# Chatit-cloud/BEE2BEE

Measured on NVIDIA H100. Metric: decode_tokens_per_sec, higher is better.
Workload: dtype bf16

## Files before the change

csrc/attention_tc.cu:

```cuda
#include "kernels.h"

#include <cuda.h>
#include <cuda_fp8.h>

#include <cstdlib>
#include <type_traits>

#include "common.cuh"
#include "launch.cuh"
#include "wgmma.cuh"

namespace b2b {

int make_tmap_shared(CUtensorMap* m, const void* ptr, uint64_t rows, uint64_t cols, uint64_t ld, uint32_t box_rows,
                     int elt_bytes);

namespace {

constexpr int APAGE = 64;
constexpr int ATC_CONSUMERS = 256;
constexpr int ATC_THREADS = ATC_CONSUMERS + 32;
constexpr float LOG2E = 1.4426950408889634f;

struct AttnTcParams {
  __nv_bfloat16* out;
  const int* block_table;
  const int* q_start;
  const int* q_len;
  const int* kv_len;
  int max_pages, n_q, n_kv, window;
  float softcap;
  int splits, ws_rows;
  float* ws;
  uint8_t* q_out8;
  uint8_t* q_sf;
  int q_bn;
};

template <int D>
struct AtcCfg {
  static constexpr int BKV = 64;
  static constexpr int kQBytes = 128 * D * 2;
  static constexpr int kKVBytes = BKV * D * 2;
  static constexpr int kSmemBytes = kQBytes + 4 * kKVBytes + 256;
};

template <int D, bool SOFTCAP>
__global__ void __launch_bounds__(ATC_THREADS, 1)
attn_prefill_tc_kernel(const __grid_constant__ CUtensorMap tm_q, const __grid_constant__ CUtensorMap tm_k,
                       const __grid_constant__ CUtensorMap tm_v, const AttnTcParams p, const int G, const int QB) {
  using Cfg = AtcCfg<D>;
  constexpr int BKV = Cfg::BKV;
  constexpr int DB = D / 64;

  extern __shared__ __align__(1024) uint8_t smem[];
  if ((smem_u32(smem) & 1023u) != 0u) __trap();
  uint8_t* q_s = smem;
  uint8_t* k_s = q_s + Cfg::kQBytes;
  uint8_t* v_s = k_s + 2 * Cfg::kKVBytes;
  uint64_t* bars = reinterpret_cast<uint64_t*>(v_s + 2 * Cfg::kKVBytes);
  uint64_t* q_full = bars + 0;
  uint64_t* k_full = bars + 1;
  uint64_t* v_full = bars + 3;
  uint64_t* k_empty = bars + 5;
  uint64_t* v_empty = bars + 7;

  const int warp = threadIdx.x >> 5, lane = threadIdx.x & 31;
  if (threadIdx.x == ATC_CONSUMERS) {
    mbar_init(q_full, 1);
    for (int i = 0; i < 2; ++i) {
      mbar_init(&k_full[i], 1); mbar_init(&v_full[i], 1);
      mbar_init(&k_empty[i], ATC_CONSUMERS / 32); mbar_init(&v_empty[i], ATC_CONSUMERS / 32);
    }
    fence_barrier_init();
    tma_prefetch_desc(&tm_q); tma_prefetch_desc(&tm_k); tma_prefetch_desc(&tm_v);
  }
  __syncthreads();

  pdl_launch_dependents();
  pdl_wait();
  const int seq = blockIdx.z, kvh = blockIdx.y;
  const bool split_mode = p.splits > 1;
  const int qblk = split_mode ? 0 : gridDim.x - 1 - blockIdx.x;
  const int qlen = p.q_len[seq], kvlen = p.kv_len[seq];
  const int q0 = qblk * QB;
  bool active = q0 < qlen;
  const int nq_here = min(QB, qlen - q0);
  const int qtok0 = p.q_start[seq] + q0;
  const int pos0 = kvlen - qlen + q0;
  const int kv_hi = min(kvlen, pos0 + nq_here);
  const int kv_lo = p.window > 0 ? max(0, pos0 - p.window + 1) : 0;
  int t_lo = kv_lo / BKV, t_hi = (kv_hi + BKV - 1) / BKV;
  if (active && split_mode) {
    const int per = (t_hi - t_lo + p.splits - 1) / p.splits;
    t_lo = min(t_hi, t_lo + static_cast<int>(blockIdx.x) * per);
    t_hi = min(t_hi, t_lo + per);
    if (t_hi <= t_lo) {
      if (threadIdx.x < G) {
        float* w = p.ws + (((static_cast<size_t>(seq) * p.n_kv + kvh) * p.splits + blockIdx.x) * p.ws_rows + threadIdx.x) * (D + 2);
        for (int c = 0; c < D; ++c) w[c] = 0.f;
        w[D] = -INFINITY;
        w[D + 1] = 0.f;
      }
      active = false;
    }
  }
  const int nt = t_hi - t_lo;
  if (!active) return;

  if (warp == ATC_CONSUMERS / 32) {
    if (lane == 0) {
      mbar_arrive_expect_tx(q_full, Cfg::kQBytes);
      for (int g = 0; g < G; ++g)
        for (int c = 0; c < DB; ++c)
          tma_load_2d(q_s + c * (128 * 128) + g * QB * 128, &tm_q, q_full, (kvh * G + g) * D + c * 64, qtok0);
      const int* bt = p.block_table + static_cast<size_t>(seq) * p.max_pages;
      for (int n = 0; n < nt; ++n) {
        const int s = n & 1;
        const uint32_t ph = static_cast<uint32_t>((n >> 1) & 1);
        const int page = bt[t_lo + n];
        mbar_wait(&k_empty[s], ph ^ 1u);
        mbar_arrive_expect_tx(&k_full[s], Cfg::kKVBytes);
#pragma unroll
        for (int c = 0; c < DB; ++c)
          tma_load_2d(k_s + s * Cfg::kKVBytes + c * (BKV * 128), &tm_k, &k_full[s], kvh * D + c * 64, page * APAGE);
        mbar_wait(&v_empty[s], ph ^ 1u);
        mbar_arrive_expect_tx(&v_full[s], Cfg::kKVBytes);
#pragma unroll
        for (int c = 0; c < DB; ++c)
          tma_load_2d(v_s + s * Cfg::kKVBytes + c * (BKV * 128), &tm_v, &v_full[s], kvh * D + c * 64, page * APAGE);
      }
    }
    return;
  }

  const int wg = warp >> 2;
  const int ra = wg * 64 + (warp & 3) * 16 + (lane >> 2);
  int gq[2], iq[2], qpos[2];
  bool valid[2];
#pragma unroll
  for (int h = 0; h < 2; ++h) {
    const int row = ra + 8 * h;
    gq[h] = row / QB;
    iq[h] = row % QB;
    valid[h] = (gq[h] < G) && (iq[h] < nq_here);
    qpos[h] = pos0 + iq[h];
  }
  const float cap = p.softcap;
  const float inv_cap = SOFTCAP ? 1.f / cap : 0.f;
  float m_ref[2] = {-INFINITY, -INFINITY}, l[2] = {0.f, 0.f};
  float o[D / 2];
#pragma unroll
  for (int e = 0; e < D / 2; ++e) o[e] = 0.f;
  auto release = [&](uint64_t* bar) {
    __syncwarp();
    if (lane == 0) mbar_arrive(bar);
  };

  mbar_wait(q_full, 0);
  auto tile = [&](int n, auto masked) {
    const int t = t_lo + n, s = n & 1;
    const uint32_t ph = static_cast<uint32_t>((n >> 1) & 1);
    float sc[BKV / 2];
#pragma unroll
    for (int e = 0; e < BKV / 2; ++e) sc[e] = 0.f;
    mbar_wait(&k_full[s], ph);
    wgmma_fence();
#pragma unroll
    for (int kk = 0; kk < D / 16; ++kk) {
      const uint64_t a = make_sw128_kmajor_desc(smem_u32(q_s + (kk / 4) * (128 * 128) + wg * 64 * 128)) +
                         static_cast<uint64_t>((kk % 4) * 2);
      const uint64_t b = make_sw128_kmajor_desc(smem_u32(k_s + s * Cfg::kKVBytes + (kk / 4) * (BKV * 128))) +
                         static_cast<uint64_t>((kk % 4) * 2);
      Wgmma<BKV>::bf16_ss(sc, a, b, kk > 0 ? 1u : 0u);
    }
    wgmma_commit();
    wgmma_wait<0>();
    wgmma_fence_regs(sc);
    release(&k_empty[s]);

    float mrow[2] = {-INFINITY, -INFINITY};
#pragma unroll
    for (int e = 0; e < BKV / 2; ++e) {
      const int h = (e >> 1) & 1;
      float v = sc[e];
      if constexpr (SOFTCAP) v = cap * tanhf(v * inv_cap);
      v *= LOG2E;
      if constexpr (decltype(masked)::value) {
        const int kvpos = t * BKV + (e >> 2) * 8 + 2 * (lane & 3) + (e & 1);
        const bool ok = valid[h] && kvpos <= qpos[h] && kvpos < kvlen && (p.window <= 0 || kvpos > qpos[h] - p.window);
        v = ok ? v : -INFINITY;
      }
      sc[e] = v;
      mrow[h] = fmaxf(mrow[h], v);
    }
    float alpha[2], mr[2];
#pragma unroll
    for (int h = 0; h < 2; ++h) {
      mrow[h] = fmaxf(mrow[h], __shfl_xor_sync(0xffffffffu, mrow[h], 1));
      mrow[h] = fmaxf(mrow[h], __shfl_xor_sync(0xffffffffu, mrow[h], 2));
      alpha[h] = 1.f;
      if (mrow[h] > m_ref[h] + 8.f || (m_ref[h] == -INFINITY && mrow[h] > -INFINITY)) {
        alpha[h] = (m_ref[h] == -INFINITY) ? 0.f : exp2f(m_ref[h] - mrow[h]);
        m_ref[h] = mrow[h];
      }
      mr[h] = (m_ref[h] == -INFINITY) ? 0.f : m_ref[h];
    }
#pragma unroll
    for (int e = 0; e < D / 2; ++e) o[e] *= alpha[(e >> 1) & 1];
    uint32_t pa[BKV / 16][4];
    float lsum[2] = {0.f, 0.f};
#pragma unroll
    for (int e = 0; e < BKV / 2; e += 2) {
      const int h = (e >> 1) & 1;
      const float p0 = exp2f(sc[e] - mr[h]), p1 = exp2f(sc[e + 1] - mr[h]);
      lsum[h] += p0 + p1;
      const __nv_bfloat162 hv = __floats2bfloat162_rn(p0, p1);
      pa[e / 8][(e % 8) / 2] = *reinterpret_cast<const uint32_t*>(&hv);
    }
    l[0] = l[0] * alpha[0] + lsum[0];
    l[1] = l[1] * alpha[1] + lsum[1];
    mbar_wait(&v_full[s], ph);
    wgmma_fence_regs(o);
    wgmma_fence();
#pragma unroll
    for (int kk = 0; kk < BKV / 16; ++kk) {
      const uint64_t b = make_sw128_mnmajor_desc(smem_u32(v_s + s * Cfg::kKVBytes + kk * (16 * 128)), BKV * 128);
      Wgmma<D>::bf16_rs_tb(o, pa[kk], b, 1u);
    }
    wgmma_commit();
    wgmma_wait<0>();
    wgmma_fence_regs(o);
    release(&v_empty[s]);
  };

  for (int n = 0; n < nt; ++n) {
    const int t = t_lo + n;
    const bool full = nq_here == QB && (t + 1) * BKV - 1 <= pos0 && (t + 1) * BKV <= kvlen &&
                      (p.window <= 0 || t * BKV > pos0 + nq_here - 1 - p.window);
    if (full) tile(n, std::false_type{}); else tile(n, std::true_type{});
  }

#pragma unroll
  for (int h = 0; h < 2; ++h) {
    l[h] += __shfl_xor_sync(0xffffffffu, l[h], 1);
    l[h] += __shfl_xor_sync(0xffffffffu, l[h], 2);
  }
  const int c2 = 2 * (lane & 3);
#pragma unroll
  for (int h = 0; h < 2; ++h) {
    const float inv = l[h] > 0.f ? 1.f / l[h] : 0.f;
    const int tok = qtok0 + iq[h], head = kvh * G + gq[h];
    if (split_mode) {
      if (valid[h]) {
        float* wsrow = p.ws + (((static_cast<size_t>(seq) * p.n_kv + kvh) * p.splits + blockIdx.x) * p.ws_rows + gq[h]) * (D + 2);
        if ((lane & 3) == 0) {
          wsrow[D] = (m_ref[h] == -INFINITY) ? -INFINITY : m_ref[h] * 0.6931471805599453f;
          wsrow[D + 1] = l[h];
        }
#pragma unroll
        for (int j = 0; j < D / 8; ++j)
          *reinterpret_cast<float2*>(wsrow + 8 * j + c2) = make_float2(o[4 * j + 2 * h], o[4 * j + 2 * h + 1]);
      }
    } else if (p.q_out8 != nullptr) {
      const int ldq = p.n_q * D;
#pragma unroll
      for (int b = 0; b < D / 32; ++b) {
        float v[8];
        float amax = 0.f;
#pragma unroll
        for (int jj = 0; jj < 4; ++jj) {
          v[2 * jj] = bf16_round(o[4 * (4 * b + jj) + 2 * h] * inv);
          v[2 * jj + 1] = bf16_round(o[4 * (4 * b + jj) + 2 * h + 1] * inv);
          amax = fmaxf(amax, fmaxf(fabsf(v[2 * jj]), fabsf(v[2 * jj + 1])));
        }
        amax = fmaxf(amax, __shfl_xor_sync(0xffffffffu, amax, 1));
        amax = fmaxf(amax, __shfl_xor_sync(0xffffffffu, amax, 2));
        const uint32_t u = __float_as_uint(amax * (1.f / 448.f));
        int ex = static_cast<int>(u >> 23) - 127 + ((u & 0x7FFFFFu) ? 1 : 0);
        ex = max(-126, min(127, ex));
        const float scl = __uint_as_float(static_cast<uint32_t>(127 - ex) << 23);
        if (valid[h]) {
          const int feat = head * D + 32 * b;
          uint8_t* q8 = p.q_out8 + static_cast<size_t>(tok) * ldq + feat;
#pragma unroll
          for (int jj = 0; jj < 4; ++jj) {
            const uint16_t lo = __nv_cvt_float_to_fp8(v[2 * jj] * scl, __NV_SATFINITE, __NV_E4M3);
            const uint16_t hi = __nv_cvt_float_to_fp8(v[2 * jj + 1] * scl, __NV_SATFINITE, __NV_E4M3);
            *reinterpret_cast<uint16_t*>(q8 + 8 * jj + c2) = static_cast<uint16_t>(lo | (hi << 8));
          }
          if ((lane & 3) == 0) {
            const int tile_i = tok / p.q_bn, n = tok - tile_i * p.q_bn, rr = n & 127;
            p.q_sf[(static_cast<size_t>(tile_i) * (ldq >> 7) + (feat >> 7)) * (p.q_bn > 128 ? 1024 : 512) + (n >> 7) * 512 +
                   (rr & 31) * 16 + (rr >> 5) * 4 + ((feat >> 5) & 3)] = static_cast<uint8_t>(ex + 127);
          }
        }
      }
    } else if (valid[h]) {
      __nv_bfloat16* dst = p.out + (static_cast<size_t>(tok) * p.n_q + head) * D;
#pragma unroll
      for (int j = 0; j < D / 8; ++j)
        *reinterpret_cast<__nv_bfloat162*>(dst + 8 * j + c2) =
            __floats2bfloat162_rn(o[4 * j + 2 * h] * inv, o[4 * j + 2 * h + 1] * inv);
    }
  }
}

template <int D, bool SOFTCAP>
int launch_tc_cap(const CUtensorMap& tq, const CUtensorMap& tk, const CUtensorMap& tv, const AttnTcParams& p, int G, int QB,
                  int seqs, int qblocks, cudaStream_t s) {
  using Cfg = AtcCfg<D>;
  static bool set[64] = {};
  int dev = 0;
  cudaGetDevice(&dev);
  if (dev < 64 && !set[dev]) {
    cudaError_t e = cudaFuncSetAttribute(attn_prefill_tc_kernel<D, SOFTCAP>, cudaFuncAttributeMaxDynamicSharedMemorySize,
                                         Cfg::kSmemBytes);
    if (e != cudaSuccess) return static_cast<int>(e);
    set[dev] = true;
  }
  return static_cast<int>(launch_kernel(attn_prefill_tc_kernel<D, SOFTCAP>,
                                        dim3(p.splits > 1 ? p.splits : qblocks, p.n_kv, seqs), dim3(ATC_THREADS),
                                        Cfg::kSmemBytes, s, 1, tq, tk, tv, p, G, QB));
}

template <int D>
int launch_tc(const CUtensorMap& tq, const CUtensorMap& tk, const CUtensorMap& tv, const AttnTcParams& p, int G, int QB,
              int seqs, int qblocks, cudaStream_t s) {
  return p.softcap > 0.f ? launch_tc_cap<D, true>(tq, tk, tv, p, G, QB, seqs, qblocks, s)
                         : launch_tc_cap<D, false>(tq, tk, tv, p, G, QB, seqs, qblocks, s);
}

}

bool attention_tc_supported(int n_q, int n_kv, int head_dim) {
  if (n_kv <= 0 || n_q % n_kv) return false;
  const int G = n_q / n_kv;
  if (G != 1 && G != 2 && G != 4 && G != 8 && G != 16) return false;
  return head_dim == 64 || head_dim == 128 || head_dim == 256;
}

int launch_attention_tc(const void* q, const void* k_cache, const void* v_cache, void* out, const int* block_table,
                        const int* q_start, const int* q_len, const int* kv_len, int seqs, int max_q, int max_pages,
                        int n_tokens, int n_pages, int n_q, int n_kv, int head_dim, int window, float softcap,
                        int splits, float* ws, void* q_out8, void* q_sf, int q_bn, cudaStream_t s) {
  if (!attention_tc_supported(n_q, n_kv, head_dim)) return -2;
  const int G = n_q / n_kv, QB = 128 / G;
  CUtensorMap tq, tk, tv;
  int r = make_tmap_shared(&tq, q, static_cast<uint64_t>(n_tokens), static_cast<uint64_t>(n_q) * head_dim,
                           static_cast<uint64_t>(n_q) * head_dim, static_cast<uint32_t>(QB), 2);
  if (r) return r;
  const uint64_t kv_rows = static_cast<uint64_t>(n_pages) * APAGE, kv_cols = static_cast<uint64_t>(n_kv) * head_dim;
  if ((r = make_tmap_shared(&tk, k_cache, kv_rows, kv_cols, kv_cols, APAGE, 2))) return r;
  if ((r = make_tmap_shared(&tv, v_cache, kv_rows, kv_cols, kv_cols, APAGE, 2))) return r;
  AttnTcParams p;
  p.out = static_cast<__nv_bfloat16*>(out);
  p.block_table = block_table; p.q_start = q_start; p.q_len = q_len; p.kv_len = kv_len;
  p.max_pages = max_pages; p.n_q = n_q; p.n_kv = n_kv; p.window = window; p.softcap = softcap;
  p.splits = (max_q == 1 && splits > 1 && ws != nullptr) ? splits : 1;
  p.ws = ws;
  p.ws_rows = attn_rows(G, 1);
  p.q_out8 = p.splits > 1 ? nullptr : static_cast<uint8_t*>(q_out8);
  p.q_sf = static_cast<uint8_t*>(q_sf);
  p.q_bn = q_bn > 0 ? q_bn : 32;
  if (q_out8 != nullptr && p.splits > 1) return -8;
  const int qblocks = (max_q + QB - 1) / QB;
  int rc;
  switch (head_dim) {
    case 64: rc = launch_tc<64>(tq, tk, tv, p, G, QB, seqs, qblocks, s); break;
    case 128: rc = launch_tc<128>(tq, tk, tv, p, G, QB, seqs, qblocks, s); break;
    case 256: rc = launch_tc<256>(tq, tk, tv, p, G, QB, seqs, qblocks, s); break;
    default: return -3;
  }
  if (rc == 0 && p.splits > 1)
    rc = launch_attention_merge(out, q_start, q_len, ws, seqs, n_q, n_kv, head_dim, p.splits, s);
  return rc;
}

}
```

csrc/binding.cpp:

```cpp
#include <ATen/cuda/CUDAContext.h>
#include <c10/cuda/CUDAGuard.h>
#include <torch/extension.h>

#include "gemm_tc.cuh"
#include "kernels.h"
#include "launch.cuh"
#include "peer.h"

using at::Tensor;
using OptT = c10::optional<Tensor>;

namespace {

inline cudaStream_t cur_stream() { return at::cuda::getCurrentCUDAStream().stream(); }

inline void check(int err, const char* what) {
  if (err != 0) {
    const char* msg = err > 0 ? cudaGetErrorString(static_cast<cudaError_t>(err)) : "invalid argument";
    TORCH_CHECK(false, what, " failed: code ", err, " (", msg, ")");
  }
}
template <typename T>
inline T* ptr_or_null(const OptT& t) {
  return (t.has_value() && t->defined()) ? reinterpret_cast<T*>(t->data_ptr()) : nullptr;
// ... 192 lines not shown
                                   static_cast<int>(x.numel() / h), h, static_cast<float>(eps), with_rms ? 1 : 0,
                                   cur_stream()),
        "quant_fp8_rows");
}

void quant_mxfp8_rows(const Tensor& x, const Tensor& q, const Tensor& sf, int64_t bn, double eps, int64_t with_rms,
                      const OptT& sumsq_out) {
  check_bf16(x, "x");
  TORCH_CHECK(q.scalar_type() == at::kFloat8_e4m3fn && q.is_contiguous() && sf.scalar_type() == at::kByte &&
                  sf.is_contiguous(), "quant_mxfp8_rows: q must be float8_e4m3fn, sf uint8");
  c10::cuda::CUDAGuard guard(x.device());
  const int h = static_cast<int>(x.size(-1));
  const int tokens = static_cast<int>(x.numel() / h);
  TORCH_CHECK(sf.numel() >= ((tokens + bn - 1) / bn) * (h / 128) * (bn > 128 ? 1024 : 512), "quant_mxfp8_rows: sf too small");
  check(b2b::launch_quant_mxfp8_rows(x.data_ptr(), q.data_ptr(), sf.data_ptr(), tokens, h, static_cast<int>(bn),
                                     static_cast<float>(eps), static_cast<int>(with_rms), ptr_or_null<float>(sumsq_out),
                                     cur_stream()),
        "quant_mxfp8_rows");
}

void flag_wait(int64_t flag, int64_t epoch, int64_t delta) {
  check(b2b::launch_flag_wait(as_ptr<const uint32_t>(flag), as_ptr<const uint32_t>(epoch),
                              static_cast<uint32_t>(delta), cur_stream()),
        "flag_wait");
}
void decode_advance(const Tensor& positions, const Tensor& kv_len, const Tensor& slots, const Tensor& q_len,
                    const Tensor& block_table) {
  c10::cuda::CUDAGuard guard(positions.device());
  check(b2b::launch_decode_advance(reinterpret_cast<int*>(positions.data_ptr()), reinterpret_cast<int*>(kv_len.data_ptr()),
                                   reinterpret_cast<int*>(slots.data_ptr()),
                                   reinterpret_cast<const int*>(q_len.data_ptr()),
                                   reinterpret_cast<const int*>(block_table.data_ptr()),
                                   static_cast<int>(block_table.size(1)), static_cast<int>(positions.numel()),
                                   cur_stream()),
        "decode_advance");
}
void flag_signal(int64_t flag, int64_t epoch, int64_t bump_epoch, int64_t ack_flag) {
  check(b2b::launch_flag_signal(as_ptr<uint32_t>(flag), as_ptr<uint32_t>(epoch), as_ptr<uint32_t>(bump_epoch),
                                as_ptr<uint32_t>(ack_flag), cur_stream()),
        "flag_signal");
}

static int64_t g_attn_tc_min_q = 2;
void set_attn_tc_min_q(int64_t v) { g_attn_tc_min_q = v; }
int64_t get_attn_tc_min_q() { return g_attn_tc_min_q; }

bool attention_uses_tc(int64_t max_q, int64_t n_q, int64_t n_kv, int64_t head_dim, int64_t use_tc) {
  if (use_tc == 0 || g_attn_tc_min_q <= 0 ||
      !b2b::attention_tc_supported(static_cast<int>(n_q), static_cast<int>(n_kv), static_cast<int>(head_dim)))
    return false;
  return use_tc > 0 || max_q == 1 || max_q >= g_attn_tc_min_q;
}

void attention(const Tensor& q, const Tensor& k_cache, const Tensor& v_cache, const Tensor& out,
               const Tensor& block_table, const Tensor& q_start, const Tensor& q_len, const Tensor& kv_len,
               const OptT& ws, int64_t max_q, int64_t n_q, int64_t n_kv, int64_t head_dim, int64_t window,
               double softcap, int64_t splits, int64_t use_tc, int64_t fq_out, int64_t fq_sf, int64_t fq_bn) {
  check_bf16(q, "q");
  c10::cuda::CUDAGuard guard(q.device());
  TORCH_CHECK(block_table.scalar_type() == at::kInt && q_len.scalar_type() == at::kInt, "int32 metadata expected");
  const int seqs = static_cast<int>(q_len.size(0));
  const bool tc = attention_uses_tc(max_q, n_q, n_kv, head_dim, use_tc);
  if (splits > 1 && (!tc || max_q == 1)) {
    TORCH_CHECK(ws.has_value(), "split-KV needs a workspace");
    const int64_t R = b2b::attn_rows(static_cast<int>(n_q / n_kv), 1);
    TORCH_CHECK(ws->numel() >= seqs * n_kv * splits * R * (head_dim + 2), "attention workspace too small");
  }
  if (tc) {
    check(b2b::launch_attention_tc(q.data_ptr(), k_cache.data_ptr(), v_cache.data_ptr(), out.data_ptr(),
                                   reinterpret_cast<const int*>(block_table.data_ptr()),
                                   reinterpret_cast<const int*>(q_start.data_ptr()),
                                   reinterpret_cast<const int*>(q_len.data_ptr()),
                                   reinterpret_cast<const int*>(kv_len.data_ptr()), seqs, static_cast<int>(max_q),
                                   static_cast<int>(block_table.size(1)), static_cast<int>(q.size(0)),
                                   static_cast<int>(k_cache.size(0)), static_cast<int>(n_q), static_cast<int>(n_kv),
                                   static_cast<int>(head_dim), static_cast<int>(window), static_cast<float>(softcap),
                                   static_cast<int>(splits), ptr_or_null<float>(ws), as_ptr<void>(fq_out), as_ptr<void>(fq_sf),
                                   static_cast<int>(fq_bn), cur_stream()),
          "attention_tc");
    return;
  }
  TORCH_CHECK(fq_out == 0, "fused output quantisation needs the tensor-core attention kernel");
  check(b2b::launch_attention(q.data_ptr(), k_cache.data_ptr(), v_cache.data_ptr(), out.data_ptr(),
                              reinterpret_cast<const int*>(block_table.data_ptr()),
                              reinterpret_cast<const int*>(q_start.data_ptr()),
                              reinterpret_cast<const int*>(q_len.data_ptr()),
                              reinterpret_cast<const int*>(kv_len.data_ptr()), ptr_or_null<float>(ws), seqs,
                              static_cast<int>(max_q), static_cast<int>(block_table.size(1)), static_cast<int>(n_q),
                              static_cast<int>(n_kv), static_cast<int>(head_dim), static_cast<int>(window),
                              static_cast<float>(softcap), static_cast<int>(splits), cur_stream()),
        "attention");
}

void sample(const Tensor& logits, const OptT& seen, const Tensor& out_tokens, int64_t peer_tokens,
            int64_t history, const OptT& hist_pos, int64_t hist_stride, int64_t vocab, double softcap,
            const OptT& temperature, const OptT& top_p,
            const OptT& rep_penalty, const OptT& seeds, const OptT& step, int64_t signal_flag, int64_t signal_epoch,
            int64_t done_counter, int64_t row_map) {
  TORCH_CHECK(logits.is_cuda() && logits.scalar_type() == at::kFloat && logits.stride(1) == 1, "logits: fp32");
  c10::cuda::CUDAGuard guard(logits.device());
  int* hp = ptr_or_null<int>(hist_pos);
  check(b2b::launch_sample(reinterpret_cast<const float*>(logits.data_ptr()), ptr_or_null<uint32_t>(seen),
                           reinterpret_cast<int*>(out_tokens.data_ptr()), as_ptr<int>(peer_tokens),
                           as_ptr<int>(history), hp, hp, static_cast<int>(hist_stride),
                           static_cast<int>(logits.size(0)), static_cast<int>(vocab > 0 ? vocab : logits.size(1)),
                           static_cast<int>(logits.stride(0)), static_cast<float>(softcap),
                           ptr_or_null<const float>(temperature), ptr_or_null<const float>(top_p),
                           ptr_or_null<const float>(rep_penalty), ptr_or_null<const uint32_t>(seeds),
                           ptr_or_null<const uint32_t>(step), as_ptr<uint32_t>(signal_flag),
                           as_ptr<uint32_t>(signal_epoch), as_ptr<uint32_t>(done_counter), as_ptr<const int>(row_map),
                           cur_stream()),
        "sample");
}

int64_t sample_cluster_size(int64_t batch, int64_t vocab) {
  int dev = 0, sms = 0;
  check(static_cast<int>(cudaGetDevice(&dev)), "cudaGetDevice");
  check(static_cast<int>(cudaDeviceGetAttribute(&sms, cudaDevAttrMultiProcessorCount, dev)), "cudaDeviceGetAttribute");
  return b2b::sample_cluster_size(static_cast<int>(batch), static_cast<int>(vocab), sms);
}

void set_decode_state(const Tensor& positions, const Tensor& kv_len, const Tensor& q_len, int64_t row_map, int64_t kvlen,
                      int64_t n) {
  c10::cuda::CUDAGuard guard(positions.device());
  check(b2b::launch_set_decode_state(reinterpret_cast<int*>(positions.data_ptr()), reinterpret_cast<int*>(kv_len.data_ptr()),
                                     reinterpret_cast<int*>(q_len.data_ptr()), as_ptr<const int>(row_map),
                                     as_ptr<const int>(kvlen), static_cast<int>(n), cur_stream()),
        "set_decode_state");
}

void fetch_window(int64_t history, int64_t hist_stride, int64_t cursors, int64_t rows, int64_t width, int64_t out,
// ... 32 lines not shown
  return static_cast<int64_t>(reinterpret_cast<uintptr_t>(p));
}
void ipc_close(int64_t p) { check(b2b::ipc_close(as_ptr<void>(p)), "cudaIpcCloseMemHandle"); }
void enable_peer_access(int64_t dev, int64_t peer) {
  check(b2b::enable_peer_access(static_cast<int>(dev), static_cast<int>(peer)), "cudaDeviceEnablePeerAccess");
}
bool can_access_peer(int64_t dev, int64_t peer) {
  return b2b::can_access_peer(static_cast<int>(dev), static_cast<int>(peer)) != 0;
}
void memcpy_peer(int64_t dst, int64_t dst_dev, int64_t src, int64_t src_dev, int64_t bytes) {
  check(b2b::memcpy_peer_async(as_ptr<void>(dst), static_cast<int>(dst_dev), as_ptr<const void>(src),
                               static_cast<int>(src_dev), static_cast<size_t>(bytes), cur_stream()),
        "cudaMemcpyPeerAsync");
}
std::pair<int64_t, int64_t> host_ring_alloc(int64_t bytes) {
  void *h = nullptr, *d = nullptr;
  check(b2b::host_ring_alloc(static_cast<size_t>(bytes), &h, &d), "cudaHostAlloc");
  return {static_cast<int64_t>(reinterpret_cast<uintptr_t>(h)), static_cast<int64_t>(reinterpret_cast<uintptr_t>(d))};
}
void host_ring_free(int64_t h) { check(b2b::host_ring_free(as_ptr<void>(h)), "cudaFreeHost"); }

Tensor tensor_from_ptr(int64_t p, std::vector<int64_t> sizes, const std::string& dtype, int64_t device) {
  at::ScalarType st = dtype == "bf16" ? at::kBFloat16 : dtype == "f32" ? at::kFloat : dtype == "i32" ? at::kInt
                      : dtype == "u8" ? at::kByte : at::kLong;
  auto opts = at::TensorOptions().dtype(st);
  opts = device >= 0 ? opts.device(at::kCUDA, static_cast<c10::DeviceIndex>(device)) : opts.device(at::kCPU);
  return at::from_blob(as_ptr<void>(p), sizes, opts);
}

}

PYBIND11_MODULE(TORCH_EXTENSION_NAME, m) {
  m.doc() = "bee2bee_b200 native sm_90a kernels + NVLink peer-memory runtime";
  m.def("gemm", &gemm);
  m.def("gemm_max_splitk", &gemm_max_splitk);
  m.def("gemm_resolve", &gemm_resolve, py::arg("bn"), py::arg("epi"), py::arg("k"), py::arg("fp8"), py::arg("stages"),
        py::arg("splitk"));
  m.def("init_kernels", &init_kernels);
  m.def("set_pdl", &set_pdl);
  m.def("get_pdl", &get_pdl);
  m.def("rmsnorm", &rmsnorm);
  m.def("layernorm", &layernorm);
  m.def("embed", &embed);
  m.def("kv_append", &kv_append);
  m.def("add", &add);
  m.def("quant_fp8_rows", &quant_fp8_rows);
  m.def("quant_mxfp8_rows", &quant_mxfp8_rows);
  m.def("flag_wait", &flag_wait);
  m.def("flag_signal", &flag_signal);
  m.def("decode_advance", &decode_advance);
  m.def("attention", &attention);
  m.def("attention_uses_tc", &attention_uses_tc, py::arg("max_q"), py::arg("n_q"), py::arg("n_kv"), py::arg("head_dim"),
        py::arg("use_tc") = -1);
  m.def("set_attn_tc_min_q", &set_attn_tc_min_q);
  m.def("get_attn_tc_min_q", &get_attn_tc_min_q);
  m.def("sample", &sample);
  m.def("sample_cluster_size", &sample_cluster_size, py::arg("batch"), py::arg("vocab"));
  m.def("mark_seen", &mark_seen);
  m.def("set_decode_state", &set_decode_state);
  m.def("fetch_window", &fetch_window);
  m.def("set_wait_policy", &set_wait_policy);
  m.def("peer_alloc", &peer_alloc);
  m.def("peer_free", &peer_free);
  m.def("ipc_export", &ipc_export);
  m.def("ipc_import", &ipc_import);
  m.def("ipc_close", &ipc_close);
  m.def("enable_peer_access", &enable_peer_access);
  m.def("can_access_peer", &can_access_peer);
  m.def("memcpy_peer", &memcpy_peer);
  m.def("host_ring_alloc", &host_ring_alloc);
  m.def("host_ring_free", &host_ring_free);
  m.def("tensor_from_ptr", &tensor_from_ptr);
}
```

csrc/gemm_tc.cu:

```cuda
#include "gemm_tc.cuh"

#include <cuda_fp8.h>

#include <cstdio>
#include <map>
#include <mutex>
#include <tuple>

#include "common.cuh"
#include "launch.cuh"
#include "wgmma.cuh"

namespace b2b {

constexpr int BM = 128;
constexpr int BK = 64;
constexpr int ROW_BYTES = 128;
constexpr int A_STAGE_BYTES = BM * ROW_BYTES;
constexpr int GEMM_CONSUMERS = 256;
constexpr int GEMM_THREADS = GEMM_CONSUMERS + 32;

template <int BN>
struct GemmCfg {
  static constexpr int kStages = (BN <= 32) ? 5 : (BN == 64 ? 4 : (BN == 128 ? 6 : 4));
  static constexpr int kStageBytes = A_STAGE_BYTES + BN * ROW_BYTES;
  static constexpr int kSfaBytes = 512;
  static constexpr int kSfbBytes = BN > 128 ? 1024 : 512;
  static constexpr int kSfBytes = kSfaBytes + kSfbBytes;
  static constexpr int kAccBytes = BM * (BN + 4) * 4 + BN * 256;
  __host__ __device__ static constexpr int ring_bytes(int stages) {
    return stages * kStageBytes > kAccBytes ? stages * kStageBytes : kAccBytes;
  }
  __host__ __device__ static constexpr int smem_bytes(int stages) {
    return ring_bytes(stages) + 1024  + 256  + BN * 12 + stages * kSfBytes;
  }
  static constexpr int kSmemBytes = smem_bytes(kStages);
};

__device__ __forceinline__ float gelu_tanh(float x) {
  const float k0 = 0.7978845608028654f, k1 = 0.044715f;
  float u = k0 * (x + k1 * x * x * x);
  return 0.5f * x * (1.f + tanhf(u));
}
__device__ __forceinline__ float silu(float x) { return x / (1.f + __expf(-x)); }

__device__ __forceinline__ unsigned long long gtime() {
  unsigned long long t;
  asm volatile("mov.u64 %0, %%globaltimer;" : "=l"(t));
  return t;
}
#define B2B_DBG(slot)                                                                                          \
  do {                                                                                                         \
    if (p.dbg != nullptr)                                                                                      \
      p.dbg[((blockIdx.z * gridDim.y + blockIdx.y) * gridDim.x + blockIdx.x) * 8 + (slot)] = gtime();          \
  } while (0)

__device__ __forceinline__ void epi_bar_sync() { asm volatile("bar.sync 1, 128;" ::: "memory"); }
__device__ __forceinline__ void consumer_bar_sync() { asm volatile("bar.sync 2, 256;" ::: "memory"); }
__device__ __forceinline__ float ue8m0(uint8_t e) { return __uint_as_float(static_cast<uint32_t>(e) << 23); }

template <int BN, int EPI, int QM>
__global__ void __launch_bounds__(GEMM_THREADS, 1) gemm_tc_kernel(const __grid_constant__ CUtensorMap tmap_w,
// ... 554 lines not shown
                                        dim3(GEMM_THREADS), Cfg::smem_bytes(p.stages), stream, static_cast<unsigned>(p.splitk), tw, tx, p));
}

template <int BN>
static int launch_bn(const GemmParams& p, const CUtensorMap& tw, const CUtensorMap& tx, cudaStream_t stream) {
#define B2B_EPI_CASE(E)                                                                              \
  case E:                                                                                            \
    if (p.fp8 && p.sfa != nullptr) {                                                                 \
      if constexpr (BN >= 32) return launch_bn_epi<BN, E, 2>(p, tw, tx, stream);                     \
      else return -7;              \
    }                                                                                                \
    return p.fp8 ? launch_bn_epi<BN, E, 1>(p, tw, tx, stream) : launch_bn_epi<BN, E, 0>(p, tw, tx, stream);
  switch (p.epi) {
    B2B_EPI_CASE(EPI_PLAIN)
    B2B_EPI_CASE(EPI_RESIDUAL)
    B2B_EPI_CASE(EPI_GLU)
    B2B_EPI_CASE(EPI_QKV_ROPE)
    B2B_EPI_CASE(EPI_GELU)
    default: return -4;
  }
#undef B2B_EPI_CASE
}

template <int BN, int EPI, int QM>
static int set_attr_one() {
  return static_cast<int>(cudaFuncSetAttribute(gemm_tc_kernel<BN, EPI, QM>, cudaFuncAttributeMaxDynamicSharedMemorySize,
                                               GemmCfg<BN>::kSmemBytes));
}
template <int BN, int EPI>
static int set_attr_epi() {
  int r = 0;
  if ((r = set_attr_one<BN, EPI, 0>()) || (r = set_attr_one<BN, EPI, 1>())) return r;
  if constexpr (BN >= 32) r = set_attr_one<BN, EPI, 2>();
  return r;
}
template <int BN>
static int set_attr_bn() {
  int r = 0;
  if ((r = set_attr_epi<BN, EPI_PLAIN>()) || (r = set_attr_epi<BN, EPI_RESIDUAL>()) || (r = set_attr_epi<BN, EPI_GLU>()) ||
      (r = set_attr_epi<BN, EPI_QKV_ROPE>()) || (r = set_attr_epi<BN, EPI_GELU>()))
    return r;
  return 0;
}
int gemm_tc_init() {
  int r = 0;
  if ((r = set_attr_bn<16>())) return r;
  if ((r = set_attr_bn<32>())) return r;
  if ((r = set_attr_bn<64>())) return r;
  if ((r = set_attr_bn<128>())) return r;
  if ((r = set_attr_bn<256>())) return r;
  return get_encode() ? 0 : -1;
}

int gemm_tc_default_stages(int bn) {
  switch (bn) {
    case 16: return GemmCfg<16>::kStages;
    case 32: return GemmCfg<32>::kStages;
    case 64: return GemmCfg<64>::kStages;
    case 128: return GemmCfg<128>::kStages;
    default: return GemmCfg<256>::kStages;
  }
}

int gemm_tc_max_splitk(int bn, int epi, int stages) {
  int ring;
  const int dflt = gemm_tc_default_stages(bn);
  if (stages <= 0 || stages > dflt) stages = dflt;
  if (stages < 2) stages = 2;
  switch (bn) {
    case 16: ring = GemmCfg<16>::ring_bytes(stages); break;
    case 32: ring = GemmCfg<32>::ring_bytes(stages); break;
    case 64: ring = GemmCfg<64>::ring_bytes(stages); break;
    case 128: ring = GemmCfg<128>::ring_bytes(stages); break;
    default: ring = GemmCfg<256>::ring_bytes(stages); break;
  }
  int best = 1;
  for (int s = 2; s <= 8 && bn / s >= 2; s *= 2) {
    const int need = s * 128 * (bn / s + 4) * 4 + (epi == EPI_GLU ? (bn / s) * 256 : 0);
    if (need <= ring) best = s;
  }
  return best;
}

int gemm_tc_resolve(int bn, int epi, int k, int fp8, int stages, int splitk, int* stages_out, int* splitk_out) {
  if (bn != 16 && bn != 32 && bn != 64 && bn != 128 && bn != 256) return -3;
  if (fp8 == 2 && bn < 32) return -7;
  const int dflt = gemm_tc_default_stages(bn);
  if (stages <= 0 || stages > dflt) stages = dflt;
  if (stages < 2) stages = 2;
  if (splitk < 1) splitk = 1;
  if (splitk > 8) splitk = 8;
  const int smax = gemm_tc_max_splitk(bn, epi, stages);
  if (splitk > smax) splitk = smax;
  const int nkb = k / (fp8 ? ROW_BYTES : ROW_BYTES / 2);
  if (splitk > nkb) splitk = nkb;
  while (splitk & (splitk - 1)) --splitk;
  *stages_out = stages;
  *splitk_out = splitk;
  return 0;
}

int launch_gemm_tc(const GemmParams& p_in, const void* w, const void* x, int bn, cudaStream_t stream) {
  GemmParams p = p_in;
  const int elt = p.fp8 ? 1 : 2;
  const int bke = ROW_BYTES / elt;
  if (p.n_out % BM != 0 || p.k % bke != 0 || p.m_tok <= 0) return -2;
// ... 31 lines not shown
```

csrc/kernels.h:

```cpp
#pragma once
#include <cuda_runtime.h>
#include <stddef.h>
#include <stdint.h>

namespace b2b {

int launch_rmsnorm(const void* x, const void* gamma, const void* residual, void* out, float* rstd_out, int tokens,
                   int h, float eps, int gemma_plus_one, cudaStream_t s);
int launch_layernorm(const void* x, const void* gamma, const void* beta, void* out, int tokens, int h, float eps,
                     cudaStream_t s);
int launch_embed(const int* ids, const void* table, const void* pos_table, const int* positions, void* out, int tokens,
                 int h, int vocab, float scale, const uint32_t* tok_flag, const uint32_t* tok_epoch, const uint32_t* pf_flag,
                 const uint32_t* pf_need, cudaStream_t s);
int launch_kv_append(const void* qkv, void* q_out, void* k_cache, void* v_cache, const int* slots, int tokens,
                     int q_dim, int kv_dim, float q_scale, cudaStream_t s);
int launch_add(const void* a, const void* b, void* out, size_t n, cudaStream_t s);
int launch_quant_fp8_rows(const void* x, void* q, float* scale_out, int tokens, int h, float eps, int with_rms,
                          cudaStream_t s);
int launch_quant_mxfp8_rows(const void* x, void* q, void* sf, int tokens, int h, int bn, float eps, int with_rms,
                            float* sumsq_out, cudaStream_t s);
int launch_flag_wait(const uint32_t* flag, const uint32_t* epoch, uint32_t delta, cudaStream_t s);
int launch_decode_advance(int* positions, int* kv_len, int* slots, const int* q_len, const int* block_table,
                          int max_pages, int n, cudaStream_t s);
int launch_flag_signal(uint32_t* flag, uint32_t* epoch, uint32_t* bump_epoch, uint32_t* ack_flag, cudaStream_t s);

int launch_attention(const void* q, const void* k_cache, const void* v_cache, void* out, const int* block_table,
                     const int* q_start, const int* q_len, const int* kv_len, float* ws, int seqs, int max_q,
                     int max_pages, int n_q, int n_kv, int head_dim, int window, float softcap, int splits,
                     cudaStream_t s);
int attn_rows(int G, int QB);
bool attention_tc_supported(int n_q, int n_kv, int head_dim);
int launch_attention_tc(const void* q, const void* k_cache, const void* v_cache, void* out, const int* block_table,
                        const int* q_start, const int* q_len, const int* kv_len, int seqs, int max_q, int max_pages,
                        int n_tokens, int n_pages, int n_q, int n_kv, int head_dim, int window, float softcap,
                        int splits, float* ws, void* q_out8, void* q_sf, int q_bn, cudaStream_t s);
int launch_attention_merge(void* out, const int* q_start, const int* q_len, const float* ws, int seqs, int n_q, int n_kv,
                           int head_dim, int splits, cudaStream_t s);
int attention_init();

int launch_sample(const float* logits, uint32_t* seen, int* out_tokens, int* peer_tokens, int* history,
                  const int* hist_pos, int* hist_pos_out, int hist_stride, int batch, int vocab, int ld, float softcap,
                  const float* temperature, const float* top_p, const float* rep_penalty, const uint32_t* seeds,
                  const uint32_t* step, uint32_t* signal_flag, uint32_t* signal_epoch, uint32_t* done_counter,
                  const int* row_map, cudaStream_t s);
int sample_cluster_size(int batch, int vocab, int sms);
int launch_set_decode_state(int* positions, int* kv_len, int* q_len, const int* row_map, const int* kvlen, int n,
                            cudaStream_t s);
struct FlagWait { const uint32_t* flag; uint32_t target; uint32_t pad; };
int launch_fetch_window(const int* history, int hist_stride, const int* cursors, int rows, int width, int* out,
                        const FlagWait* waits, int n_waits, int* status, cudaStream_t s);
int launch_mark_seen(const int* ids, const int* seq_of, uint32_t* seen, int n, int vocab, cudaStream_t s);

int set_wait_policy_gemm(uint32_t* abort_word, unsigned long long limit_ns);
int set_wait_policy_elementwise(uint32_t* abort_word, unsigned long long limit_ns);

int gemm_tc_max_splitk(int bn, int epi, int stages);
int gemm_tc_init();

}
```

Baseline: 4744.

## Add single-warpgroup decode attention kernel sized to co-reside with O-proj GEMM

Templates the tensor-core attention body on warpgroup count and adds a decode variant with one consumer warpgroup (64 query rows), a single KV stage, and a 128-register cap. Decode calls (max_q==1, no split) route to it, so two attention CTAs plus an O-projection GEMM CTA can fit on one SM together with PDL overlap. It also adds footprint introspection bindings. The trade-off is no double buffering of K/V and the loss of split-KV in decode, which can leave SMs underfilled for long contexts with few sequences.

```diff
diff --git a/csrc/attention_tc.cu b/csrc/attention_tc.cu
--- a/csrc/attention_tc.cu
+++ b/csrc/attention_tc.cu
@@ -18,8 +18,6 @@
 namespace {
 
 constexpr int APAGE = 64;
-constexpr int ATC_CONSUMERS = 256;
-constexpr int ATC_THREADS = ATC_CONSUMERS + 32;
 constexpr float LOG2E = 1.4426950408889634f;
 
 struct AttnTcParams {
@@ -37,40 +35,49 @@
   int q_bn;
 };
 
-template <int D>
+template <int D, int NWG>
 struct AtcCfg {
   static constexpr int BKV = 64;
-  static constexpr int kQBytes = 128 * D * 2;
+  static constexpr int kRows = 64 * NWG;
+  static constexpr int kConsumers = 128 * NWG;
+  static constexpr int kThreads = kConsumers + 32;
+  static constexpr int kStages = NWG == 2 ? 2 : 1;
+  static constexpr int kQBytes = kRows * D * 2;
   static constexpr int kKVBytes = BKV * D * 2;
-  static constexpr int kSmemBytes = kQBytes + 4 * kKVBytes + 256;
+  static constexpr int kSmemBytes = kQBytes + 2 * kStages * kKVBytes + 256;
 };
-
-template <int D, bool SOFTCAP>
-__global__ void __launch_bounds__(ATC_THREADS, 1)
-attn_prefill_tc_kernel(const __grid_constant__ CUtensorMap tm_q, const __grid_constant__ CUtensorMap tm_k,
-                       const __grid_constant__ CUtensorMap tm_v, const AttnTcParams p, const int G, const int QB) {
-  using Cfg = AtcCfg<D>;
+constexpr int ATC_DECODE_MAXNREG = 128;
+static_assert(2 * (AtcCfg<128, 1>::kSmemBytes + 1024) + 109184 + 1024 <= 233472,
+              "two D = 128 decode CTAs and one O-proj CTA must share an SM's shared memory");
+
+template <int D, bool SOFTCAP, int NWG>
+__device__ __forceinline__ void attn_tc_body(const CUtensorMap& tm_q, const CUtensorMap& tm_k, const CUtensorMap& tm_v,
+                                             const AttnTcParams& p, const int G, const int QB) {
+  using Cfg = AtcCfg<D, NWG>;
   constexpr int BKV = Cfg::BKV;
   constexpr int DB = D / 64;
+  constexpr int ROWS = Cfg::kRows;
+  constexpr int CONSUMERS = Cfg::kConsumers;
+  constexpr int STAGES = Cfg::kStages;
 
   extern __shared__ __align__(1024) uint8_t smem[];
   if ((smem_u32(smem) & 1023u) != 0u) __trap();
   uint8_t* q_s = smem;
   uint8_t* k_s = q_s + Cfg::kQBytes;
-  uint8_t* v_s = k_s + 2 * Cfg::kKVBytes;
-  uint64_t* bars = reinterpret_cast<uint64_t*>(v_s + 2 * Cfg::kKVBytes);
+  uint8_t* v_s = k_s + STAGES * Cfg::kKVBytes;
+  uint64_t* bars = reinterpret_cast<uint64_t*>(v_s + STAGES * Cfg::kKVBytes);
   uint64_t* q_full = bars + 0;
   uint64_t* k_full = bars + 1;
-  uint64_t* v_full = bars + 3;
-  uint64_t* k_empty = bars + 5;
-  uint64_t* v_empty = bars + 7;
+  uint64_t* v_full = k_full + STAGES;
+  uint64_t* k_empty = v_full + STAGES;
+  uint64_t* v_empty = k_empty + STAGES;
 
   const int warp = threadIdx.x >> 5, lane = threadIdx.x & 31;
-  if (threadIdx.x == ATC_CONSUMERS) {
+  if (threadIdx.x == CONSUMERS) {
     mbar_init(q_full, 1);
-    for (int i = 0; i < 2; ++i) {
+    for (int i = 0; i < STAGES; ++i) {
       mbar_init(&k_full[i], 1); mbar_init(&v_full[i], 1);
-      mbar_init(&k_empty[i], ATC_CONSUMERS / 32); mbar_init(&v_empty[i], ATC_CONSUMERS / 32);
+      mbar_init(&k_empty[i], CONSUMERS / 32); mbar_init(&v_empty[i], CONSUMERS / 32);
     }
     fence_barrier_init();
     tma_prefetch_desc(&tm_q); tma_prefetch_desc(&tm_k); tma_prefetch_desc(&tm_v);
@@ -80,7 +87,7 @@
   pdl_launch_dependents();
   pdl_wait();
   const int seq = blockIdx.z, kvh = blockIdx.y;
-  const bool split_mode = p.splits > 1;
+  const bool split_mode = NWG == 2 && p.splits > 1;
   const int qblk = split_mode ? 0 : gridDim.x - 1 - blockIdx.x;
   const int qlen = p.q_len[seq], kvlen = p.kv_len[seq];
   const int q0 = qblk * QB;
@@ -108,16 +115,16 @@
   const int nt = t_hi - t_lo;
   if (!active) return;
 
-  if (warp == ATC_CONSUMERS / 32) {
+  if (warp == CONSUMERS / 32) {
     if (lane == 0) {
       mbar_arrive_expect_tx(q_full, Cfg::kQBytes);
       for (int g = 0; g < G; ++g)
         for (int c = 0; c < DB; ++c)
-          tma_load_2d(q_s + c * (128 * 128) + g * QB * 128, &tm_q, q_full, (kvh * G + g) * D + c * 64, qtok0);
+          tma_load_2d(q_s + c * (ROWS * 128) + g * QB * 128, &tm_q, q_full, (kvh * G + g) * D + c * 64, qtok0);
       const int* bt = p.block_table + static_cast<size_t>(seq) * p.max_pages;
       for (int n = 0; n < nt; ++n) {
-        const int s = n & 1;
-        const uint32_t ph = static_cast<uint32_t>((n >> 1) & 1);
+        const int s = n % STAGES;
+        const uint32_t ph = static_cast<uint32_t>((n / STAGES) & 1);
         const int page = bt[t_lo + n];
         mbar_wait(&k_empty[s], ph ^ 1u);
         mbar_arrive_expect_tx(&k_full[s], Cfg::kKVBytes);
@@ -159,8 +166,8 @@
 
   mbar_wait(q_full, 0);
   auto tile = [&](int n, auto masked) {
-    const int t = t_lo + n, s = n & 1;
-    const uint32_t ph = static_cast<uint32_t>((n >> 1) & 1);
+    const int t = t_lo + n, s = n % STAGES;
+    const uint32_t ph = static_cast<uint32_t>((n / STAGES) & 1);
     float sc[BKV / 2];
 #pragma unroll
     for (int e = 0; e < BKV / 2; ++e) sc[e] = 0.f;
@@ -168,7 +175,7 @@
     wgmma_fence();
 #pragma unroll
     for (int kk = 0; kk < D / 16; ++kk) {
-      const uint64_t a = make_sw128_kmajor_desc(smem_u32(q_s + (kk / 4) * (128 * 128) + wg * 64 * 128)) +
+      const uint64_t a = make_sw128_kmajor_desc(smem_u32(q_s + (kk / 4) * (ROWS * 128) + wg * 64 * 128)) +
                          static_cast<uint64_t>((kk % 4) * 2);
       const uint64_t b = make_sw128_kmajor_desc(smem_u32(k_s + s * Cfg::kKVBytes + (kk / 4) * (BKV * 128))) +
                          static_cast<uint64_t>((kk % 4) * 2);
@@ -236,9 +243,13 @@
 
   for (int n = 0; n < nt; ++n) {
     const int t = t_lo + n;
-    const bool full = nq_here == QB && (t + 1) * BKV - 1 <= pos0 && (t + 1) * BKV <= kvlen &&
-                      (p.window <= 0 || t * BKV > pos0 + nq_here - 1 - p.window);
-    if (full) tile(n, std::false_type{}); else tile(n, std::true_type{});
+    if constexpr (NWG == 2) {
+      const bool full = nq_here == QB && (t + 1) * BKV - 1 <= pos0 && (t + 1) * BKV <= kvlen &&
+                        (p.window <= 0 || t * BKV > pos0 + nq_here - 1 - p.window);
+      if (full) tile(n, std::false_type{}); else tile(n, std::true_type{});
+    } else {
+      tile(n, std::true_type{});
+    }
   }
 
 #pragma unroll
@@ -307,28 +318,68 @@
 }
 
 template <int D, bool SOFTCAP>
-int launch_tc_cap(const CUtensorMap& tq, const CUtensorMap& tk, const CUtensorMap& tv, const AttnTcParams& p, int G, int QB,
-                  int seqs, int qblocks, cudaStream_t s) {
-  using Cfg = AtcCfg<D>;
+__global__ void __launch_bounds__(AtcCfg<D, 2>::kThreads, 1)
+attn_prefill_tc_kernel(const __grid_constant__ CUtensorMap tm_q, const __grid_constant__ CUtensorMap tm_k,
+                       const __grid_constant__ CUtensorMap tm_v, const AttnTcParams p, const int G, const int QB) {
+  attn_tc_body<D, SOFTCAP, 2>(tm_q, tm_k, tm_v, p, G, QB);
+}
+
+template <int D, bool SOFTCAP>
+__global__ void __maxnreg__(ATC_DECODE_MAXNREG)
+attn_decode_tc_kernel(const __grid_constant__ CUtensorMap tm_q, const __grid_constant__ CUtensorMap tm_k,
+                      const __grid_constant__ CUtensorMap tm_v, const AttnTcParams p, const int G, const int QB) {
+  attn_tc_body<D, SOFTCAP, 1>(tm_q, tm_k, tm_v, p, G, QB);
+}
+
+template <int D, bool SOFTCAP, int NWG>
+constexpr auto atc_kernel() {
+  if constexpr (NWG == 2) return attn_prefill_tc_kernel<D, SOFTCAP>;
+  else return attn_decode_tc_kernel<D, SOFTCAP>;
+}
+
+template <int D, bool SOFTCAP, int NWG>
+int set_smem_attr() {
   static bool set[64] = {};
   int dev = 0;
   cudaGetDevice(&dev);
-  if (dev < 64 && !set[dev]) {
-    cudaError_t e = cudaFuncSetAttribute(attn_prefill_tc_kernel<D, SOFTCAP>, cudaFuncAttributeMaxDynamicSharedMemorySize,
-                                         Cfg::kSmemBytes);
-    if (e != cudaSuccess) return static_cast<int>(e);
-    set[dev] = true;
-  }
-  return static_cast<int>(launch_kernel(attn_prefill_tc_kernel<D, SOFTCAP>,
-                                        dim3(p.splits > 1 ? p.splits : qblocks, p.n_kv, seqs), dim3(ATC_THREADS),
+  if (dev < 64 && set[dev]) return 0;
+  cudaError_t e = cudaFuncSetAttribute(atc_kernel<D, SOFTCAP, NWG>(), cudaFuncAttributeMaxDynamicSharedMemorySize,
+                                       AtcCfg<D, NWG>::kSmemBytes);
+  if (e == cudaSuccess && dev < 64) set[dev] = true;
+  return static_cast<int>(e);
+}
+
+template <int D, bool SOFTCAP, int NWG>
+int launch_tc_cap(const CUtensorMap& tq, const CUtensorMap& tk, const CUtensorMap& tv, const AttnTcParams& p, int G, int QB,
+                  int seqs, int qblocks, cudaStream_t s) {
+  using Cfg = AtcCfg<D, NWG>;
+  if (int e = set_smem_attr<D, SOFTCAP, NWG>()) return e;
+  return static_cast<int>(launch_kernel(atc_kernel<D, SOFTCAP, NWG>(),
+                                        dim3(p.splits > 1 ? p.splits : qblocks, p.n_kv, seqs), dim3(Cfg::kThreads),
                                         Cfg::kSmemBytes, s, 1, tq, tk, tv, p, G, QB));
 }
 
-template <int D>
+template <int D, int NWG>
 int launch_tc(const CUtensorMap& tq, const CUtensorMap& tk, const CUtensorMap& tv, const AttnTcParams& p, int G, int QB,
               int seqs, int qblocks, cudaStream_t s) {
-  return p.softcap > 0.f ? launch_tc_cap<D, true>(tq, tk, tv, p, G, QB, seqs, qblocks, s)
-                         : launch_tc_cap<D, false>(tq, tk, tv, p, G, QB, seqs, qblocks, s);
+  return p.softcap > 0.f ? launch_tc_cap<D, true, NWG>(tq, tk, tv, p, G, QB, seqs, qblocks, s)
+                         : launch_tc_cap<D, false, NWG>(tq, tk, tv, p, G, QB, seqs, qblocks, s);
+}
+
+template <int D, bool SOFTCAP>
+int decode_footprint_d(KernelFootprint* f) {
+  using Cfg = AtcCfg<D, 1>;
+  if (int e = set_smem_attr<D, SOFTCAP, 1>()) return e;
+  cudaFuncAttributes a{};
+  cudaError_t e = cudaFuncGetAttributes(&a, attn_decode_tc_kernel<D, SOFTCAP>);
+  if (e == cudaSuccess)
+    e = cudaOccupancyMaxActiveBlocksPerMultiprocessor(&f->blocks_per_sm, attn_decode_tc_kernel<D, SOFTCAP>,
+                                                      Cfg::kThreads, Cfg::kSmemBytes);
+  f->regs = a.numRegs;
+  f->threads = Cfg::kThreads;
+  f->smem = static_cast<int>(a.sharedSizeBytes) + Cfg::kSmemBytes;
+  f->local_bytes = static_cast<int>(a.localSizeBytes);
+  return static_cast<int>(e);
 }
 
 }
@@ -340,12 +391,26 @@
   return head_dim == 64 || head_dim == 128 || head_dim == 256;
 }
 
+bool attention_decode_supported(int max_q, int n_q, int n_kv, int head_dim, int splits) {
+  return max_q == 1 && splits <= 1 && attention_tc_supported(n_q, n_kv, head_dim) && n_q / n_kv <= 8 &&
+         head_dim <= 128;
+}
+
+int attention_decode_footprint(int head_dim, int softcap, KernelFootprint* f) {
+  switch (head_dim) {
+    case 64: return softcap ? decode_footprint_d<64, true>(f) : decode_footprint_d<64, false>(f);
+    case 128: return softcap ? decode_footprint_d<128, true>(f) : decode_footprint_d<128, false>(f);
+    default: return -3;
+  }
+}
+
 int launch_attention_tc(const void* q, const void* k_cache, const void* v_cache, void* out, const int* block_table,
                         const int* q_start, const int* q_len, const int* kv_len, int seqs, int max_q, int max_pages,
                         int n_tokens, int n_pages, int n_q, int n_kv, int head_dim, int window, float softcap,
-                        int splits, float* ws, void* q_out8, void* q_sf, int q_bn, cudaStream_t s) {
+                        int splits, float* ws, void* q_out8, void* q_sf, int q_bn, bool decode, cudaStream_t s) {
   if (!attention_tc_supported(n_q, n_kv, head_dim)) return -2;
-  const int G = n_q / n_kv, QB = 128 / G;
+  if (decode && !attention_decode_supported(max_q, n_q, n_kv, head_dim, splits)) return -2;
+  const int G = n_q / n_kv, QB = (decode ? 64 : 128) / G;
   CUtensorMap tq, tk, tv;
   int r = make_tmap_shared(&tq, q, static_cast<uint64_t>(n_tokens), static_cast<uint64_t>(n_q) * head_dim,
                            static_cast<uint64_t>(n_q) * head_dim, static_cast<uint32_t>(QB), 2);
@@ -366,10 +431,18 @@
   if (q_out8 != nullptr && p.splits > 1) return -8;
   const int qblocks = (max_q + QB - 1) / QB;
   int rc;
+  if (decode) {
+    switch (head_dim) {
+      case 64: rc = launch_tc<64, 1>(tq, tk, tv, p, G, QB, seqs, qblocks, s); break;
+      case 128: rc = launch_tc<128, 1>(tq, tk, tv, p, G, QB, seqs, qblocks, s); break;
+      default: return -3;
+    }
+    return rc;
+  }
   switch (head_dim) {
-    case 64: rc = launch_tc<64>(tq, tk, tv, p, G, QB, seqs, qblocks, s); break;
-    case 128: rc = launch_tc<128>(tq, tk, tv, p, G, QB, seqs, qblocks, s); break;
-    case 256: rc = launch_tc<256>(tq, tk, tv, p, G, QB, seqs, qblocks, s); break;
+    case 64: rc = launch_tc<64, 2>(tq, tk, tv, p, G, QB, seqs, qblocks, s); break;
+    case 128: rc = launch_tc<128, 2>(tq, tk, tv, p, G, QB, seqs, qblocks, s); break;
+    case 256: rc = launch_tc<256, 2>(tq, tk, tv, p, G, QB, seqs, qblocks, s); break;
     default: return -3;
   }
   if (rc == 0 && p.splits > 1)
diff --git a/csrc/binding.cpp b/csrc/binding.cpp
--- a/csrc/binding.cpp
+++ b/csrc/binding.cpp
@@ -268,6 +268,41 @@
   return use_tc > 0 || max_q == 1 || max_q >= g_attn_tc_min_q;
 }
 
+bool attention_uses_decode_kernel(int64_t max_q, int64_t n_q, int64_t n_kv, int64_t head_dim, int64_t splits,
+                                  int64_t use_tc) {
+  return use_tc < 0 && attention_uses_tc(max_q, n_q, n_kv, head_dim, use_tc) &&
+         b2b::attention_decode_supported(static_cast<int>(max_q), static_cast<int>(n_q), static_cast<int>(n_kv),
+                                         static_cast<int>(head_dim), static_cast<int>(splits));
+}
+
+static py::dict footprint_dict(const b2b::KernelFootprint& f) {
+  py::dict d;
+  d["regs"] = f.regs;
+  d["threads"] = f.threads;
+  d["smem"] = f.smem;
+  d["local_bytes"] = f.local_bytes;
+  d["blocks_per_sm"] = f.blocks_per_sm;
+  int dev = 0, regs_sm = 0, smem_sm = 0, reserved = 0;
+  cudaGetDevice(&dev);
+  cudaDeviceGetAttribute(&regs_sm, cudaDevAttrMaxRegistersPerMultiprocessor, dev);
+  cudaDeviceGetAttribute(&smem_sm, cudaDevAttrMaxSharedMemoryPerMultiprocessor, dev);
+  cudaDeviceGetAttribute(&reserved, cudaDevAttrReservedSharedMemoryPerBlock, dev);
+  d["regs_per_sm"] = regs_sm;
+  d["smem_per_sm"] = smem_sm;
+  d["reserved_smem_per_block"] = reserved;
+  return d;
+}
+py::dict attention_decode_footprint(int64_t head_dim, bool softcap) {
+  b2b::KernelFootprint f{};
+  check(b2b::attention_decode_footprint(static_cast<int>(head_dim), softcap ? 1 : 0, &f), "attention_decode_footprint");
+  return footprint_dict(f);
+}
+py::dict gemm_footprint(int64_t bn, int64_t epi, int64_t fp8) {
+  b2b::KernelFootprint f{};
+  check(b2b::gemm_tc_footprint(static_cast<int>(bn), static_cast<int>(epi), static_cast<int>(fp8), &f), "gemm_footprint");
+  return footprint_dict(f);
+}
+
 void attention(const Tensor& q, const Tensor& k_cache, const Tensor& v_cache, const Tensor& out,
                const Tensor& block_table, const Tensor& q_start, const Tensor& q_len, const Tensor& kv_len,
                const OptT& ws, int64_t max_q, int64_t n_q, int64_t n_kv, int64_t head_dim, int64_t window,
@@ -277,6 +312,7 @@
   TORCH_CHECK(block_table.scalar_type() == at::kInt && q_len.scalar_type() == at::kInt, "int32 metadata expected");
   const int seqs = static_cast<int>(q_len.size(0));
   const bool tc = attention_uses_tc(max_q, n_q, n_kv, head_dim, use_tc);
+  const bool decode_kernel = attention_uses_decode_kernel(max_q, n_q, n_kv, head_dim, splits, use_tc);
   if (splits > 1 && (!tc || max_q == 1)) {
     TORCH_CHECK(ws.has_value(), "split-KV needs a workspace");
     const int64_t R = b2b::attn_rows(static_cast<int>(n_q / n_kv), 1);
@@ -292,7 +328,7 @@
                                    static_cast<int>(k_cache.size(0)), static_cast<int>(n_q), static_cast<int>(n_kv),
                                    static_cast<int>(head_dim), static_cast<int>(window), static_cast<float>(softcap),
                                    static_cast<int>(splits), ptr_or_null<float>(ws), as_ptr<void>(fq_out), as_ptr<void>(fq_sf),
-                                   static_cast<int>(fq_bn), cur_stream()),
+                                   static_cast<int>(fq_bn), decode_kernel, cur_stream()),
           "attention_tc");
     return;
   }
@@ -431,6 +467,10 @@
   m.def("attention", &attention);
   m.def("attention_uses_tc", &attention_uses_tc, py::arg("max_q"), py::arg("n_q"), py::arg("n_kv"), py::arg("head_dim"),
         py::arg("use_tc") = -1);
+  m.def("attention_uses_decode_kernel", &attention_uses_decode_kernel, py::arg("max_q"), py::arg("n_q"), py::arg("n_kv"),
+        py::arg("head_dim"), py::arg("splits") = 1, py::arg("use_tc") = -1);
+  m.def("attention_decode_footprint", &attention_decode_footprint, py::arg("head_dim"), py::arg("softcap") = false);
+  m.def("gemm_footprint", &gemm_footprint, py::arg("bn"), py::arg("epi"), py::arg("fp8"));
   m.def("set_attn_tc_min_q", &set_attn_tc_min_q);
   m.def("get_attn_tc_min_q", &get_attn_tc_min_q);
   m.def("sample", &sample);
diff --git a/csrc/gemm_tc.cu b/csrc/gemm_tc.cu
--- a/csrc/gemm_tc.cu
+++ b/csrc/gemm_tc.cu
@@ -8,6 +8,7 @@
 #include <tuple>
 
 #include "common.cuh"
+#include "kernels.h"
 #include "launch.cuh"
 #include "wgmma.cuh"
 
@@ -668,6 +669,51 @@
   return get_encode() ? 0 : -1;
 }
 
+template <int BN, int EPI, int QM>
+static int footprint_one(KernelFootprint* f) {
+  using Cfg = GemmCfg<BN>;
+  if (int r = set_attr_one<BN, EPI, QM>()) return r;
+  cudaFuncAttributes a{};
+  cudaError_t e = cudaFuncGetAttributes(&a, gemm_tc_kernel<BN, EPI, QM>);
+  if (e == cudaSuccess)
+    e = cudaOccupancyMaxActiveBlocksPerMultiprocessor(&f->blocks_per_sm, gemm_tc_kernel<BN, EPI, QM>, GEMM_THREADS,
+                                                      Cfg::kSmemBytes);
+  f->regs = a.numRegs;
+  f->threads = GEMM_THREADS;
+  f->smem = static_cast<int>(a.sharedSizeBytes) + Cfg::kSmemBytes;
+  f->local_bytes = static_cast<int>(a.localSizeBytes);
+  return static_cast<int>(e);
+}
+template <int BN>
+static int footprint_bn(int epi, int qm, KernelFootprint* f) {
+#define B2B_EPI_CASE(E)                                                                                 \
+  case E:                                                                                               \
+    if (qm == 2) {                                                                                      \
+      if constexpr (BN >= 32) return footprint_one<BN, E, 2>(f);                                        \
+      else return -7;                                                                                   \
+    }                                                                                                   \
+    return qm == 1 ? footprint_one<BN, E, 1>(f) : footprint_one<BN, E, 0>(f);
+  switch (epi) {
+    B2B_EPI_CASE(EPI_PLAIN)
+    B2B_EPI_CASE(EPI_RESIDUAL)
+    B2B_EPI_CASE(EPI_GLU)
+    B2B_EPI_CASE(EPI_QKV_ROPE)
+    B2B_EPI_CASE(EPI_GELU)
+    default: return -4;
+  }
+#undef B2B_EPI_CASE
+}
+int gemm_tc_footprint(int bn, int epi, int qm, KernelFootprint* f) {
+  switch (bn) {
+    case 16: return footprint_bn<16>(epi, qm, f);
+    case 32: return footprint_bn<32>(epi, qm, f);
+    case 64: return footprint_bn<64>(epi, qm, f);
+    case 128: return footprint_bn<128>(epi, qm, f);
+    case 256: return footprint_bn<256>(epi, qm, f);
+    default: return -3;
+  }
+}
+
 int gemm_tc_default_stages(int bn) {
   switch (bn) {
     case 16: return GemmCfg<16>::kStages;
diff --git a/csrc/kernels.h b/csrc/kernels.h
--- a/csrc/kernels.h
+++ b/csrc/kernels.h
@@ -29,11 +29,14 @@
                      int max_pages, int n_q, int n_kv, int head_dim, int window, float softcap, int splits,
                      cudaStream_t s);
 int attn_rows(int G, int QB);
+struct KernelFootprint { int regs, threads, smem, local_bytes, blocks_per_sm; };
 bool attention_tc_supported(int n_q, int n_kv, int head_dim);
+bool attention_decode_supported(int max_q, int n_q, int n_kv, int head_dim, int splits);
+int attention_decode_footprint(int head_dim, int softcap, KernelFootprint* f);
 int launch_attention_tc(const void* q, const void* k_cache, const void* v_cache, void* out, const int* block_table,
                         const int* q_start, const int* q_len, const int* kv_len, int seqs, int max_q, int max_pages,
                         int n_tokens, int n_pages, int n_q, int n_kv, int head_dim, int window, float softcap,
-                        int splits, float* ws, void* q_out8, void* q_sf, int q_bn, cudaStream_t s);
+                        int splits, float* ws, void* q_out8, void* q_sf, int q_bn, bool decode, cudaStream_t s);
 int launch_attention_merge(void* out, const int* q_start, const int* q_len, const float* ws, int seqs, int n_q, int n_kv,
                            int head_dim, int splits, cudaStream_t s);
 int attention_init();
@@ -56,5 +59,6 @@
 
 int gemm_tc_max_splitk(int bn, int epi, int stages);
 int gemm_tc_init();
+int gemm_tc_footprint(int bn, int epi, int qm, KernelFootprint* f);
 
 }
```

Result: faster. 4798 (median of 6 runs) (+1.1%).
